# dimforge/rapier

Measured on NVIDIA H100. Metric: physics steps/sec on b3d_many_pyramids (3D f32), higher is better.
Workload: dtype f32

## Files before the change

### rapier_b200/csrc/rb_solver.cuh

```cuda
#pragma once
#include "rb_collide.cuh"
#include "rb_ccd.cuh"

namespace rb {

constexpr int SB_VEC = 7;
constexpr int SB_STRIDE = SB_VEC * 4;

struct BodyState { vec3 lin, ang; pose p; sym3 ii; vec3 im; };

struct SmemBodies {
    float* s;
    RB_HD float4* row(int i, int r) const { return reinterpret_cast<float4*>(s) + i * SB_VEC + r; }
    RB_HD vec3 lin(int i) const { return xyz(*row(i, 0)); }
    RB_HD vec3 ang(int i) const { return xyz(*row(i, 1)); }
    RB_HD void set_vel(int i, vec3 l, vec3 a) const {
        float4* r0 = row(i, 0); float4* r1 = row(i, 1);
        *r0 = make_float4(l.x, l.y, l.z, r0->w);
        *r1 = make_float4(a.x, a.y, a.z, r1->w);
    }
    RB_HD pose xf(int i) const { return mkpose(mkq(*row(i, 2)), xyz(*row(i, 3))); }
    RB_HD void set_xf(int i, const pose& p) const {
        *row(i, 2) = f4(p.q);
        float4* r3 = row(i, 3);
// ... 1428 lines not shown
        }

        float4 ti4 = mu.mr(MR_TI, s);
        float ti0 = ti4.x, ti1 = ti4.y, wi = wi4.x;
        float ta0 = ti4.z, ta1 = ti4.w, wa = wi4.y;
        if (MODE == MODE_WARMSTART || (MODE != MODE_RESTITUTION && solve_friction)) {
            const FrictionJac fj = coop_get_jac(cs, s);
            if (MODE == MODE_WARMSTART) {
                ta0 = ta0 + ti0; ta1 = ta1 + ti1;
                ti0 = ti0 * P.warmstart_coeff; ti1 = ti1 * P.warmstart_coeff;
                wa = wa + wi;
                wi = wi * P.warmstart_coeff;
                friction_warmstart_jac(g1, g2, t1, t2, nc, fj, ti0, ti1, wi, v1, w1, v2, w2);
            } else {
                const float4 twd = cs.pc(CR4_TWD, s);
                float tlimit = 0.0f, wlimit = 0.0f;
#pragma unroll
                for (int kk = 0; kk < MAX_PTS; ++kk) {
                    const float ik = lane_bcast<L>(imp[kk / L], kk % L);
                    if (kk < nc) {
                        tlimit = tlimit + ik;
                        wlimit = fma_(ik, kk == 0 ? twd.x : (kk == 1 ? twd.y : (kk == 2 ? twd.z : twd.w)), wlimit);
                    }
                }
                tlimit = tlimit * dirf.w;
                wlimit = wlimit * dirf.w;
                constexpr bool relax = MODE == MODE_RELAX;
                vec3 lfc1 = zero3(), lfc2 = zero3();
                if (!relax) { lfc1 = xyz(crow(w, CR_LFC1, q0 + s)); lfc2 = xyz(crow(w, CR_LFC2, q0 + s)); }
                FrictionState f;
                f.ti0 = ti0; f.ti1 = ti1; f.wi = wi;
                friction_solve_jac(P, g1, g2, dir, t1, t2, nc, tlimit, wlimit, t1w.w, fj, trn.x, trn.y, trn.z, relax, lfc1, lfc2, f, v1,
                                   w1, v2, w2);
                ti0 = f.ti0; ti1 = f.ti1; wi = f.wi;
            }
        }
        if (active && !skip) {
#pragma unroll
            for (int j = 0; j < PPL; ++j) {
                const int k = sub + j * L;
                if (k < nc) {
                    mu.mf(MR_IMP, k, s) = imp[j];
                    if (MODE == MODE_WARMSTART) mu.mf(MR_ACC, k, s) = acc[j];
                    if (MODE == MODE_RELAX) mu.mf(MR_DIST, k, s) = dist_new[j];
                }
            }
            if (sub == 0) {
                if (MODE != MODE_RESTITUTION) {
                    mu.mr(MR_TI, s) = make_float4(ti0, ti1, ta0, ta1);
                    mu.mr(MR_WI, s) = make_float4(wi, wa, 0.0f, 0.0f);
                }
                bd.set_vel(id1 < 0 ? (wslot + 1) : id1, v1, w1);
                bd.set_vel(id2 < 0 ? (wslot + 1) : id2, v2, w2);
            }
        }
    }
}

template <int L, class B>
RB_HD void coop_stage_mode(int mode, const World& w, const B& bd, const RowView& cs, const RowView& mu, int wslot, int q0, int a, int e,
                           int tid, int nth, bool solve_friction) {
    if (mode == MODE_WARMSTART) coop_stage<L, MODE_WARMSTART>(w, bd, cs, mu, wslot, q0, a, e, tid, nth, solve_friction);
    else if (mode == MODE_BIASED) coop_stage<L, MODE_BIASED>(w, bd, cs, mu, wslot, q0, a, e, tid, nth, solve_friction);
    else if (mode == MODE_RELAX) coop_stage<L, MODE_RELAX>(w, bd, cs, mu, wslot, q0, a, e, tid, nth, solve_friction);
    else coop_stage<L, MODE_RESTITUTION>(w, bd, cs, mu, wslot, q0, a, e, tid, nth, solve_friction);
}

RB_HD void coop_bank(const RowView& mu, int s, float scale) {
    float4 im = mu.mr(MR_IMP, s), ac = mu.mr(MR_ACC, s), ti = mu.mr(MR_TI, s), wi = mu.mr(MR_WI, s);
    ac.x = ac.x + im.x; ac.y = ac.y + im.y; ac.z = ac.z + im.z; ac.w = ac.w + im.w;
    im.x = im.x * scale; im.y = im.y * scale; im.z = im.z * scale; im.w = im.w * scale;
    ti.z = ti.z + ti.x; ti.w = ti.w + ti.y; ti.x = ti.x * scale; ti.y = ti.y * scale;
    wi.y = wi.y + wi.x; wi.x = wi.x * scale;
    mu.mr(MR_IMP, s) = im; mu.mr(MR_ACC, s) = ac; mu.mr(MR_TI, s) = ti; mu.mr(MR_WI, s) = wi;
}

template <int FM, int JM>
struct HbmRows {
    static constexpr bool solve_groups = true;
    static constexpr bool generic_joints = JM != 0;
    RB_HD explicit HbmRows(const World&) {}
    template <class B>
    static RB_HD void begin(const World&, const B&) {}
    template <class B>
    static RB_HD void generate(const World& w, const B& bd, int q, int buf, int item, Cons& c) {
        cons_generate<FM>(w, bd, q, buf, item, c);
        cons_store_static<FM>(w, q, c);
        cons_store_dyn<FM>(w, q, c);
    }
    template <class B>
    static RB_HD void stage(const World& w, const B& bd, int a, int e, bool serial, int mode, bool fric, int tid, int nth, bool grp,
                            unsigned char gk) {
        if (serial) {
            if (tid == 0)
                for (int q = a; q < e; ++q) { if (grp && w.cons_key[q] != gk) continue; Cons cc; cons_load<FM>(w, q, cc); cons_sweep<FM>(w, bd, q, cc, mode, fric); cons_store_dyn<FM>(w, q, cc); }
        } else {
            for (int q = a + tid; q < e; q += nth) { if (grp && w.cons_key[q] != gk) continue; Cons cc; cons_load<FM>(w, q, cc); cons_sweep<FM>(w, bd, q, cc, mode, fric); cons_store_dyn<FM>(w, q, cc); }
        }
    }
    static RB_HD void bank(const World& w, int q, Cons& c) {
        cons_load<FM>(w, q, c);
#pragma unroll
        for (int k = 0; k < MAX_PTS; ++k)
            if (k < c.nc) { c.acc[k] = c.acc[k] + c.imp[k]; c.imp[k] = c.imp[k] * 0.0f; }
        c.ta0 = c.ta0 + c.ti0; c.ta1 = c.ta1 + c.ti1; c.ti0 = c.ti0 * 0.0f; c.ti1 = c.ti1 * 0.0f;
        c.wa = c.wa + c.wi; c.wi = c.wi * 0.0f;
        if (FM) {
#pragma unroll
            for (int k = 0; k < MAX_PTS; ++k)
                if (k < c.nc) {
                    c.pta0[k] = c.pta0[k] + c.pti0[k]; c.pta1[k] = c.pta1[k] + c.pti1[k];
                    c.pti0[k] = c.pti0[k] * 0.0f; c.pti1[k] = c.pti1[k] * 0.0f;
                }
        }
        cons_store_dyn<FM>(w, q, c);
    }
    static RB_HD void writeback(const World& w, int q, int buf, Cons& c) { cons_load<FM>(w, q, c); cons_writeback<FM>(w, q, buf, c); }
    template <class B>
    static RB_HD void update_joint(const World& w, const B& bd, int q, int sub) { if (JM) joint_update_generic(w, bd, q, sub); else joint_update(w, bd, q); }
    template <class B>
    static RB_HD void solve_joint(const World& w, const B& bd, int q, bool relax, bool warm) {
        if (JM) joint_solve_generic(w, bd, q, relax, warm); else joint_solve(w, bd, q, relax);
    }
    static RB_HD void writeback_joint(const World& w, int q) { if (JM) joint_writeback_generic(w, q); else joint_writeback(w, q); }
};

template <int L>
struct PoolRows {
    static constexpr bool solve_groups = false;
    static constexpr bool generic_joints = false;
    RowView rows, mu;
    int wslot;
    RB_HD explicit PoolRows(const World& w) {
        wslot = w.nb;
        rows.p = w.large_pool; rows.stride = w.cons_cap;
        mu.p = w.large_mut; mu.stride = w.cons_cap;
    }
    template <class B>
    RB_HD void begin(const World& w, const B& bd) const {
        bd.set_vel(wslot, zero3(), zero3());
        bd.set_xf(wslot, pident());
        w.b_eim[wslot] = make_float4(0.f, 0.f, 0.f, 0.f);
    }
    template <class B>
    RB_HD void generate(const World& w, const B& bd, int q, int buf, int item, Cons& c) const {
        cons_generate(w, bd, q, buf, item, c);
        coop_put(rows, mu, bd, q, c);
    }
    template <class B>
    RB_HD void stage(const World& w, const B& bd, int a, int e, bool serial, int mode, bool fric, int tid, int nth, bool, unsigned char) const {
        const int n = serial ? L : nth;
        if (serial && tid >= L) return;
        if (L > 1 && !serial && (e - a) * L > nth) coop_stage_mode<1>(mode, w, bd, rows, mu, wslot, 0, a, e, tid, n, fric);
        else coop_stage_mode<L>(mode, w, bd, rows, mu, wslot, 0, a, e, tid, n, fric);
    }
    RB_HD void bank(const World&, int q, Cons&) const { coop_bank(mu, q, 0.0f); }
    RB_HD void writeback(const World& w, int q, int buf, Cons& c) const {
        coop_get_for_writeback(rows, mu, q, c);
        cons_writeback(w, q, buf, c, true);
    }
    template <class B>
    static RB_HD void update_joint(const World& w, const B& bd, int q, int) { joint_update(w, bd, q); }
    template <class B>
    static RB_HD void solve_joint(const World& w, const B& bd, int q, bool relax, bool) { joint_solve(w, bd, q, relax); }
    static RB_HD void writeback_joint(const World& w, int q) { joint_writeback(w, q); }
};

template <class R, class X, class B>
RB_PHASE void solve_item(const X& ex, const World& w, const B& bd, int item, vec3 gravity) {
    const Params& P = w.prm;
    State* st = w.st;
    const int buf = st->cur;
    const bool global_ids = item == 0;
    const int b0 = w.item_body_start[item], b1 = w.item_body_start[item + 1];
    const int c0 = w.item_cons_start[item];
    const int c1 = w.item_cons_start[item + 1] < w.cons_cap ? w.item_cons_start[item + 1] : w.cons_cap;
    const int j0 = w.item_joint_start[item], j1 = w.item_joint_start[item + 1];
    const int* coff = w.item_color_off + (size_t)item * (NUM_COLORS + 1);
    const int* joff = w.item_jcolor_off + (size_t)item * (NUM_COLORS + 1);
    const int ncol = st->nused_colors, njcol = st->njused_colors;
    const int ovf = w.color_pos[COLOR_OVERFLOW], jovf = w.jcolor_pos[COLOR_OVERFLOW];
    const int tid = ex.tid(), nth = ex.nth();
    const bool grp = R::solve_groups && w.any_extra != 0;
    const unsigned char gk = (unsigned char)w.pass_key;
    const R rows(w);

    auto stage = [&](int a, int e, bool serial, int mode, bool fric) { rows.stage(w, bd, a, e, serial, mode, fric, tid, nth, grp, gk); };

    if (tid == 0) {
        w.item_flags[item] = 0;
        rows.begin(w, bd);
    }
    for (int l = b0 + tid; l < b1; l += nth) {
        int b = w.item_bodies[l];
        if (grp && w.b_key[b] != gk) continue;
        body_init(w, bd, b, global_ids ? b : l - b0, gravity);
    }
    ex.sync();
    for (int q = c0 + tid; q < c1; q += nth) {
        if (grp && w.cons_key[q] != gk) continue;
        Cons c;
        rows.generate(w, bd, q, buf, item, c);
    }
    ex.sync();

    for (int sub = 0; sub < P.num_substeps; ++sub) {
        for (int l = b0 + tid; l < b1; l += nth) {
            int b = w.item_bodies[l];
            if (grp && w.b_key[b] != gk) continue;
            body_increment(w, bd, b, global_ids ? b : l - b0);
        }
        ex.sync();
        if (j1 > j0) {
            for (int q = j0 + tid; q < j1; q += nth) { if (grp && w.j_key[q] != gk) continue; rows.update_joint(w, bd, q, sub); }
            ex.sync();
        }
        if (P.warmstart_coeff != 0.0f) {
            for (int c = 0; c < ncol; ++c) {
                int a = c0 + coff[c], e = c0 + coff[c + 1];
                if (e > c1) e = c1;
                if (a >= e) continue;
                stage(a, e, c == ovf, MODE_WARMSTART, false);
                ex.sync();
            }
        } else {
            for (int q = c0 + tid; q < c1; q += nth) {
                if (grp && w.cons_key[q] != gk) continue;
                Cons c;
                rows.bank(w, q, c);
            }
            ex.sync();
        }
        for (int pass = 0; pass < 2; ++pass) {
            const bool relax = pass == 1;
            const int iters = relax ? P.num_relax : P.num_pgs;
            const bool fric = relax || P.friction_in_bias || P.num_relax == 0;
            for (int it = 0; it < iters; ++it) {
                const bool jwarm = R::generic_joints && P.warmstart_joints && !relax && it == 0;
                for (int c = 0; c < njcol; ++c) {
                    int a = j0 + joff[c], e = j0 + joff[c + 1];
                    if (a >= e) continue;
                    if (c == jovf) {
                        if (tid == 0) for (int q = a; q < e; ++q) { if (grp && w.j_key[q] != gk) continue; rows.solve_joint(w, bd, q, relax, jwarm); }
                    } else {
                        for (int q = a + tid; q < e; q += nth) { if (grp && w.j_key[q] != gk) continue; rows.solve_joint(w, bd, q, relax, jwarm); }
                    }
                    ex.sync();
                }
                for (int c = 0; c < ncol; ++c) {
                    int a = c0 + coff[c], e = c0 + coff[c + 1];
                    if (e > c1) e = c1;
                    if (a >= e) continue;
                    stage(a, e, c == ovf, relax ? MODE_RELAX : MODE_BIASED, fric);
                    ex.sync();
                }
            }
            if (!relax) {
                for (int l = b0 + tid; l < b1; l += nth) {
                    int b = w.item_bodies[l];
                    if (grp && w.b_key[b] != gk) continue;
                    body_integrate(w, bd, b, global_ids ? b : l - b0);
                }
                ex.sync();
            }
        }
    }
    if (w.item_flags[item]) {
        for (int c = 0; c < ncol; ++c) {
            int a = c0 + coff[c], e = c0 + coff[c + 1];
            if (e > c1) e = c1;
            if (a >= e) continue;
            stage(a, e, c == ovf, MODE_RESTITUTION, false);
            ex.sync();
        }
    }
    for (int q = c0 + tid; q < c1; q += nth) { if (grp && w.cons_key[q] != gk) continue; Cons c; rows.writeback(w, q, buf, c); }
    for (int q = j0 + tid; q < j1; q += nth) { if (grp && w.j_key[q] != gk) continue; rows.writeback_joint(w, q); }
    for (int l = b0 + tid; l < b1; l += nth) {
        int b = w.item_bodies[l];
        if (grp && w.b_key[b] != gk) continue;
        body_writeback(w, bd, b, global_ids ? b : l - b0);
    }
}

RB_HD bool item_is_coop(const World& w, int item) {
    const int nbod = w.item_body_start[item + 1] - w.item_body_start[item];
    const int ncons = w.item_cons_start[item + 1] - w.item_cons_start[item];
    const int njoints = w.item_joint_start[item + 1] - w.item_joint_start[item];
    const int ovf = w.color_pos[COLOR_OVERFLOW];
    const int* coff = w.item_color_off + (size_t)item * (NUM_COLORS + 1);
    const bool has_ovf = ovf >= 0 && coff[ovf + 1] > coff[ovf];
    return item > 0 && njoints == 0 && !has_ovf && !w.prm.friction_model && ncons < 65536 && w.item_cons_start[item + 1] <= w.cons_cap &&
           coop_plan(w.coop_small_floats, nbod, ncons).ok;
}

struct CoopPipe {
    float4* buf[2];
    unsigned long long* mbar;
    float4* pool;
    const int* chunk;
    int nchunks;
    unsigned t;
    int sweep_threads;
    bool primed;
};
RB_HD RowView coop_chunk_rows(const CoopPipe& pp, int q) {
    const int o = pp.chunk[q], cnt = pp.chunk[q + 1] - o;
    RowView v;
    v.p = pp.pool + (size_t)COOP_ROWS * (o + q) - o;
    v.stride = cnt | 1;
    return v;
}
RB_HD RowView coop_slot_rows(const CoopPipe& pp, int s) {
    int lo = 0, hi = pp.nchunks - 1;
    while (lo < hi) {
        int mid = (lo + hi + 1) >> 1;
        if (pp.chunk[mid] <= s) lo = mid; else hi = mid - 1;
    }
    return coop_chunk_rows(pp, lo);
}
RB_HD void coop_pipe_issue(const CoopPipe& pp, int q, int b) {
    const int o = pp.chunk[q], cnt = pp.chunk[q + 1] - o;
    const unsigned bytes = (unsigned)(COOP_ROWS * (cnt | 1) * 16);
    mbar_expect_tx(pp.mbar + b, bytes);
    bulk_g2s(b ? pp.buf[1] : pp.buf[0], pp.pool + (size_t)COOP_ROWS * (o + q), bytes, pp.mbar + b);
}

template <int L, int MODE>
RB_PHASE void coop_sweep(const BlockCtx& ctx, const World& w, const SmemBodies& bd, const RowView& res, const RowView& mu, bool resident,
                         CoopPipe& pp, const int* s_stage, int nstages, int wslot, int c0, bool fric, bool wrap) {
    const int tid = ctx.btid, nth = pp.sweep_threads;
#ifdef RB_DEBUG
    if (w.debug_flags & 1) return;
#endif
    if (resident) {
        for (int c = 0; c < nstages; ++c) {
            const int ae = s_stage[c];
            if (tid < nth) coop_stage<L, MODE>(w, bd, res, mu, wslot, c0, ae & 0xffff, ae >> 16, tid, nth, fric);
            ctx.block_sync();
        }
        return;
    }
    if (!pp.primed && tid == 0) coop_pipe_issue(pp, 0, pp.t & 1);
    for (int q = 0; q < pp.nchunks; ++q) {
        const int o = pp.chunk[q], e = pp.chunk[q + 1];
        const int b = pp.t & 1;
        mbar_wait(pp.mbar + b, (pp.t >> 1) & 1);
        if (tid == 0) {
            if (q + 1 < pp.nchunks) coop_pipe_issue(pp, q + 1, b ^ 1);
            else if (wrap) coop_pipe_issue(pp, 0, b ^ 1);
        }
        RowView rd;
        rd.p = (b ? pp.buf[1] : pp.buf[0]) - o;
        rd.stride = (e - o) | 1;
        if (tid < nth) coop_stage<L, MODE>(w, bd, rd, mu, wslot, c0, o, e, tid, nth, fric);
        ctx.block_sync();
        pp.t += 1;
    }
    pp.primed = wrap;
}

RB_HD void coop_warmstart_bank(const Params& P, const RowView& mu, int s) {
    coop_bank(mu, s, P.warmstart_coeff);
}
RB_HD void coop_warmstart_side(const RowView& cs, const RowView& mu, int s, int side, vec3 im, vec3& v, vec3& wv) {
    const float4 dirf = cs.pc(CR4_DIRF, s), t1w = cs.pc(CR4_T1W, s), trn = cs.pc(CR4_TR, s);
    const float4 imp4 = mu.mr(MR_IMP, s), ti4 = mu.mr(MR_TI, s), wi4 = mu.mr(MR_WI, s);
    const int nc = as_int(trn.w);
    const vec3 dir = xyz(dirf), t1 = xyz(t1w);
    const vec3 t2 = cross3(dir, t1);
    const vec3 lin = had(dir, im);
    const float imp[MAX_PTS] = {imp4.x, imp4.y, imp4.z, imp4.w};
#pragma unroll
    for (int k = 0; k < MAX_PTS; ++k) {
        if (k < nc) {
            const vec3 itd = xyz(cs.pp(side == 0 ? PR4_ITD1I : PR4_ITD2A, k, s));
            v = madd3(v, lin, side == 0 ? imp[k] : -imp[k]);
            wv = madd3(wv, itd, imp[k]);
        }
    }
    const FrictionJac j = coop_get_jac(cs, s);
    const float ti0 = ti4.x, ti1 = ti4.y, wi = wi4.x;
    if (side == 0) {
        v = madd3v(v, madd3(t1 * ti0, t2, ti1), im);
        wv = madd3(madd3(wv, j.i10, ti0), j.i11, ti1);
        if (nc > 1) wv = madd3(wv, j.tw1, wi);
    } else {
        v = madd3v(v, madd3(t1 * (-ti0), t2, -ti1), im);
        wv = madd3(madd3(wv, j.i20, ti0), j.i21, ti1);
        if (nc > 1) wv = madd3(wv, j.tw2, -wi);
    }
}

template <int L>
RB_PHASE void solve_item_coop(const BlockCtx& ctx, const World& w, float* smem, int smem_floats, CoopPipe& pp, int item, vec3 gravity) {
    const Params& P = w.prm;
    State* st = w.st;
    const int buf = st->cur;
    const int b0 = w.item_body_start[item], b1 = w.item_body_start[item + 1];
    const int c0 = w.item_cons_start[item], n = w.item_cons_start[item + 1] - c0;
    const int tid = ctx.btid, nth = ctx.bsize;
    const CoopPlan plan = coop_plan(smem_floats, b1 - b0, n);
    const bool resident = plan.resident != 0;
    const int wslot = b1 - b0;
    SmemBodies bd;
    bd.s = smem;
    RowView mu;
    mu.p = reinterpret_cast<float4*>(smem + plan.body_slots * SB_STRIDE); mu.stride = plan.mstride;
    float4* cbase = mu.p + MR_COUNT * plan.mstride;
    RowView res;
    res.p = cbase; res.stride = plan.stride;
    RB_SHARED int s_stage[NUM_COLORS + 2];
    RB_SHARED int s_nstages;
    RB_SHARED int s_chunk[COOP_MAX_CHUNKS + 1];
    RB_SHARED int s_nchunks;
    RB_SHARED int s_width;
    pp.buf[0] = cbase; pp.buf[1] = cbase + (size_t)COOP_ROWS * plan.stride;
    pp.pool = w.coop_pool + (size_t)2 * COOP_ROWS * c0; pp.chunk = s_chunk; pp.primed = false;
    if (tid == 0) {
        const int* coff = w.item_color_off + (size_t)item * (NUM_COLORS + 1);
        const int ncol = st->nused_colors;
        int ns = 0;
        for (int c = 0; c < ncol; ++c)
            if (coff[c + 1] > coff[c]) s_stage[ns++] = coff[c] | (coff[c + 1] << 16);
        s_nstages = ns;
        int longest = 0;
        for (int c = 0; c < ns; ++c) longest = max2i(longest, (s_stage[c] >> 16) - (s_stage[c] & 0xffff));
        const int width = (longest * L + 31) & ~31;
        s_width = min2i(nth, max2i(width, 128));
        int nq = 0;
        if (!resident)
            for (int c = 0; c < ns; ++c)
                for (int o = s_stage[c] & 0xffff; o < (s_stage[c] >> 16); o += plan.stride) s_chunk[nq++] = o;
        s_chunk[nq] = n;
        s_nchunks = nq;
        w.item_flags[item] = 0;
        bd.set_vel(wslot, zero3(), zero3());
        bd.set_xf(wslot, pident());
        bd.set_mass(wslot, sym_zero(), zero3());
        if (!coop_plan(w.coop_small_floats, b1 - b0, n).resident) st->need_big = 1;
        atomic_add(resident ? &st->coop_resident : &st->coop_streamed, 1);
    }
#ifdef RB_DEBUG
    const bool trace = (w.debug_flags & 2) && ctx.bid == 0 && tid == 0;
    int tr = 0;
#define RB_TRACE() if (trace && tr < 32) w.dbg_times[tr++] = rb_clock()
#else
#define RB_TRACE() do {} while (0)
#endif
    RB_TRACE();
    for (int l = b0 + tid; l < b1; l += nth) body_init(w, bd, w.item_bodies[l], l - b0, gravity);
    ctx.block_sync();
    RB_TRACE();
    const int nstages = s_nstages;
    pp.nchunks = s_nchunks;
    pp.sweep_threads = s_width;
    for (int s = tid; s < n; s += nth) {
        Cons c;
        cons_generate(w, bd, c0 + s, buf, item, c);
        coop_put(resident ? res : coop_slot_rows(pp, s), mu, bd, s, c);
    }
    if (!resident) fence_async_proxy();
    ctx.block_sync();
    RB_TRACE();
    const bool bouncy_item = w.item_flags[item] != 0;
    const bool warm = P.warmstart_coeff != 0.0f;
    const int total_sweeps = P.num_substeps * ((warm ? 1 : 0) + P.num_pgs + P.num_relax) + (bouncy_item ? 1 : 0);
    int done = 0;
    for (int sub = 0; sub < P.num_substeps; ++sub) {
        for (int l = b0 + tid; l < b1; l += nth) body_increment(w, bd, w.item_bodies[l], l - b0);
        if (warm && !resident) {
            ctx.block_sync();
            ++done;
            if (sub == 0) RB_TRACE();
            coop_sweep<L, MODE_WARMSTART>(ctx, w, bd, res, mu, resident, pp, s_stage, nstages, wslot, c0, false, done < total_sweeps);
            if (sub == 0) RB_TRACE();
        } else if (warm) {
            if (sub == 0) RB_TRACE();
            for (int s = tid; s < n; s += nth) coop_warmstart_bank(P, mu, s);
            ctx.block_sync();
#ifdef RB_DEBUG
            if (!(w.debug_flags & 1))
#endif
                for (int l = tid; l < b1 - b0; l += nth) {
                    const int* adj = w.adj_list + w.adj_off[b0 + l];
                    const int cnt = w.adj_cnt[b0 + l];
                    vec3 v = bd.lin(l), wv = bd.ang(l);
                    const vec3 im = bd.im(l);
                    for (int i = 0; i < cnt; ++i) {
                        const int e = adj[i];
                        coop_warmstart_side(res, mu, e >> 1, e & 1, im, v, wv);
                    }
                    bd.set_vel(l, v, wv);
                }
            ctx.block_sync();
            if (sub == 0) RB_TRACE();
        } else {
            for (int s = tid; s < n; s += nth) coop_bank(mu, s, 0.0f);
            ctx.block_sync();
        }
        for (int pass = 0; pass < 2; ++pass) {
            const bool relax = pass == 1;
            const int iters = relax ? P.num_relax : P.num_pgs;
            const bool fric = relax || P.friction_in_bias || P.num_relax == 0;
            for (int it = 0; it < iters; ++it) {
                ++done;
                if (relax) coop_sweep<L, MODE_RELAX>(ctx, w, bd, res, mu, resident, pp, s_stage, nstages, wslot, c0, fric, done < total_sweeps);
                else coop_sweep<L, MODE_BIASED>(ctx, w, bd, res, mu, resident, pp, s_stage, nstages, wslot, c0, fric, done < total_sweeps);
                if (sub == 0) RB_TRACE();
            }
            if (!relax) {
                for (int l = b0 + tid; l < b1; l += nth) body_integrate(w, bd, w.item_bodies[l], l - b0);
                ctx.block_sync();
                if (sub == 0) RB_TRACE();
            }
        }
    }
    if (bouncy_item) coop_sweep<L, MODE_RESTITUTION>(ctx, w, bd, res, mu, resident, pp, s_stage, nstages, wslot, c0, false, false);
    RB_TRACE();
    for (int s = tid; s < n; s += nth) {
        Cons c;
        coop_get_for_writeback(resident ? res : coop_slot_rows(pp, s), mu, s, c);
        cons_writeback(w, c0 + s, buf, c, true);
    }
#ifdef RB_DEBUG
    if (w.debug_flags & 2) ctx.block_sync();
#endif
    RB_TRACE();
    for (int l = b0 + tid; l < b1; l += nth) body_writeback(w, bd, w.item_bodies[l], l - b0);
    RB_TRACE();
#undef RB_TRACE
}

}
```

Before: 3805.

## Use per-body gather warmstart for non-resident items with software-prefetched loads

Replaces the colored warmstart sweep used for non-resident (streamed) constraint items with the per-body adjacency gather, reading constraint rows straight from the global pool through a binary-searched chunk lookup. The pipeline priming moves to before the substep loop, and total_sweeps no longer counts the warmstart pass. The warmstart body loop now software-pipelines its constraint loads, fetching the next constraint's data while applying the current one. This removes one full double-buffered bulk-copy sweep per substep, at the cost of uncoalesced global reads and a binary search per adjacency entry.

```diff
diff --git a/rapier_b200/csrc/rb_solver.cuh b/rapier_b200/csrc/rb_solver.cuh
--- a/rapier_b200/csrc/rb_solver.cuh
+++ b/rapier_b200/csrc/rb_solver.cuh
@@ -1754,7 +1754,6 @@
     int nchunks;
     unsigned t;
     int sweep_threads;
-    bool primed;
 };
 RB_HD RowView coop_chunk_rows(const CoopPipe& pp, int q) {
     const int o = pp.chunk[q], cnt = pp.chunk[q + 1] - o;
@@ -1793,7 +1792,6 @@
         }
         return;
     }
-    if (!pp.primed && tid == 0) coop_pipe_issue(pp, 0, pp.t & 1);
     for (int q = 0; q < pp.nchunks; ++q) {
         const int o = pp.chunk[q], e = pp.chunk[q + 1];
         const int b = pp.t & 1;
@@ -1809,38 +1807,46 @@
         ctx.block_sync();
         pp.t += 1;
     }
-    pp.primed = wrap;
 }
 
 RB_HD void coop_warmstart_bank(const Params& P, const RowView& mu, int s) {
     coop_bank(mu, s, P.warmstart_coeff);
 }
-RB_HD void coop_warmstart_side(const RowView& cs, const RowView& mu, int s, int side, vec3 im, vec3& v, vec3& wv) {
-    const float4 dirf = cs.pc(CR4_DIRF, s), t1w = cs.pc(CR4_T1W, s), trn = cs.pc(CR4_TR, s);
-    const float4 imp4 = mu.mr(MR_IMP, s), ti4 = mu.mr(MR_TI, s), wi4 = mu.mr(MR_WI, s);
-    const int nc = as_int(trn.w);
-    const vec3 dir = xyz(dirf), t1 = xyz(t1w);
+struct WarmSide { float4 dirf, t1w, trn, itd[MAX_PTS], jac[5], imp, ti, wi; };
+RB_HD WarmSide coop_warmstart_load(const RowView& cs, const RowView& mu, int s, int side) {
+    WarmSide o;
+    o.dirf = cs.pc(CR4_DIRF, s); o.t1w = cs.pc(CR4_T1W, s); o.trn = cs.pc(CR4_TR, s);
+#pragma unroll
+    for (int k = 0; k < MAX_PTS; ++k) o.itd[k] = cs.pp(side == 0 ? PR4_ITD1I : PR4_ITD2A, k, s);
+#pragma unroll
+    for (int r = 0; r < 5; ++r) o.jac[r] = cs.pc(CR4_J3 + r, s);
+    o.imp = mu.mr(MR_IMP, s); o.ti = mu.mr(MR_TI, s); o.wi = mu.mr(MR_WI, s);
+    return o;
+}
+RB_HD void coop_warmstart_apply(const WarmSide& o, int side, vec3 im, vec3& v, vec3& wv) {
+    const int nc = as_int(o.trn.w);
+    const vec3 dir = xyz(o.dirf), t1 = xyz(o.t1w);
     const vec3 t2 = cross3(dir, t1);
     const vec3 lin = had(dir, im);
-    const float imp[MAX_PTS] = {imp4.x, imp4.y, imp4.z, imp4.w};
+    const float imp[MAX_PTS] = {o.imp.x, o.imp.y, o.imp.z, o.imp.w};
 #pragma unroll
     for (int k = 0; k < MAX_PTS; ++k) {
         if (k < nc) {
-            const vec3 itd = xyz(cs.pp(side == 0 ? PR4_ITD1I : PR4_ITD2A, k, s));
+            const vec3 itd = xyz(o.itd[k]);
             v = madd3(v, lin, side == 0 ? imp[k] : -imp[k]);
             wv = madd3(wv, itd, imp[k]);
         }
     }
-    const FrictionJac j = coop_get_jac(cs, s);
-    const float ti0 = ti4.x, ti1 = ti4.y, wi = wi4.x;
+    const float4 d = o.jac[0], e = o.jac[1], f = o.jac[2], g = o.jac[3], h = o.jac[4];
+    const float ti0 = o.ti.x, ti1 = o.ti.y, wi = o.wi.x;
     if (side == 0) {
         v = madd3v(v, madd3(t1 * ti0, t2, ti1), im);
-        wv = madd3(madd3(wv, j.i10, ti0), j.i11, ti1);
-        if (nc > 1) wv = madd3(wv, j.tw1, wi);
+        wv = madd3(madd3(wv, mk3(d.x, d.y, d.z), ti0), mk3(d.w, e.x, e.y), ti1);
+        if (nc > 1) wv = madd3(wv, mk3(g.x, g.y, g.z), wi);
     } else {
         v = madd3v(v, madd3(t1 * (-ti0), t2, -ti1), im);
-        wv = madd3(madd3(wv, j.i20, ti0), j.i21, ti1);
-        if (nc > 1) wv = madd3(wv, j.tw2, -wi);
+        wv = madd3(madd3(wv, mk3(e.z, e.w, f.x), ti0), mk3(f.y, f.z, f.w), ti1);
+        if (nc > 1) wv = madd3(wv, mk3(g.w, h.x, h.y), -wi);
     }
 }
 
@@ -1868,7 +1874,7 @@
     RB_SHARED int s_nchunks;
     RB_SHARED int s_width;
     pp.buf[0] = cbase; pp.buf[1] = cbase + (size_t)COOP_ROWS * plan.stride;
-    pp.pool = w.coop_pool + (size_t)2 * COOP_ROWS * c0; pp.chunk = s_chunk; pp.primed = false;
+    pp.pool = w.coop_pool + (size_t)2 * COOP_ROWS * c0; pp.chunk = s_chunk;
     if (tid == 0) {
         const int* coff = w.item_color_off + (size_t)item * (NUM_COLORS + 1);
         const int ncol = st->nused_colors;
@@ -1917,17 +1923,15 @@
     RB_TRACE();
     const bool bouncy_item = w.item_flags[item] != 0;
     const bool warm = P.warmstart_coeff != 0.0f;
-    const int total_sweeps = P.num_substeps * ((warm ? 1 : 0) + P.num_pgs + P.num_relax) + (bouncy_item ? 1 : 0);
+    int total_sweeps = P.num_substeps * (P.num_pgs + P.num_relax) + (bouncy_item ? 1 : 0);
+#ifdef RB_DEBUG
+    if (w.debug_flags & 1) total_sweeps = 0;
+#endif
+    if (!resident && total_sweeps > 0 && tid == 0) coop_pipe_issue(pp, 0, pp.t & 1);
     int done = 0;
     for (int sub = 0; sub < P.num_substeps; ++sub) {
         for (int l = b0 + tid; l < b1; l += nth) body_increment(w, bd, w.item_bodies[l], l - b0);
-        if (warm && !resident) {
-            ctx.block_sync();
-            ++done;
-            if (sub == 0) RB_TRACE();
-            coop_sweep<L, MODE_WARMSTART>(ctx, w, bd, res, mu, resident, pp, s_stage, nstages, wslot, c0, false, done < total_sweeps);
-            if (sub == 0) RB_TRACE();
-        } else if (warm) {
+        if (warm) {
             if (sub == 0) RB_TRACE();
             for (int s = tid; s < n; s += nth) coop_warmstart_bank(P, mu, s);
             ctx.block_sync();
@@ -1939,9 +1943,19 @@
                     const int cnt = w.adj_cnt[b0 + l];
                     vec3 v = bd.lin(l), wv = bd.ang(l);
                     const vec3 im = bd.im(l);
-                    for (int i = 0; i < cnt; ++i) {
-                        const int e = adj[i];
-                        coop_warmstart_side(res, mu, e >> 1, e & 1, im, v, wv);
+                    if (cnt > 0) {
+                        int e = adj[0], e_after = cnt > 1 ? adj[1] : 0;
+                        WarmSide next = coop_warmstart_load(resident ? res : coop_slot_rows(pp, e >> 1), mu, e >> 1, e & 1);
+                        for (int i = 0; i < cnt; ++i) {
+                            const WarmSide cur = next;
+                            const int side = e & 1;
+                            if (i + 1 < cnt) {
+                                e = e_after;
+                                if (i + 2 < cnt) e_after = adj[i + 2];
+                                next = coop_warmstart_load(resident ? res : coop_slot_rows(pp, e >> 1), mu, e >> 1, e & 1);
+                            }
+                            coop_warmstart_apply(cur, side, im, v, wv);
+                        }
                     }
                     bd.set_vel(l, v, wv);
                 }
```

Result: faster. 3922, median of 6 (+3.1%).
